# anshumang/gunrockINST

Measured on AMD Instinct MI355X. Metric: MTEPS (million traversed edges/sec) BFS R-MAT scale-24, higher is better.
Workload: dtype int32; 1 GPU; BFS idempotent direction-optimizing (traversal_mode 2), R-MAT scale-24 (a=.55 b=.2 c=.2 d=.05, 8 pairs/vertex mirrored, seed 0x6772): n=16777216, m=265395436 directed edges; sources: largest-degree + 64 seeded; search_depth_src0=7, max_degree=218420

## Files before the change

gunrockinst_amd/capi.py:

```python
import ctypes as C
import os
import subprocess

import numpy as np

_PKG = os.path.dirname(os.path.abspath(__file__))
LIB_PATH = os.environ.get("GUNROCK_LIB_PATH") or os.path.join(_PKG, "lib", "libgunrock.so")
_LIB = None

VTXID_INT = 0
SIZET_INT = 0
VALUE_INT, VALUE_UINT, VALUE_FLOAT = 0, 1, 2
SRC_MANUALLY, SRC_RANDOMIZE, SRC_LARGEST_DEGREE = 0, 1, 2

i32p = C.POINTER(C.c_int32)


class GunrockDataType(C.Structure):
    _fields_ = [("VTXID_TYPE", C.c_int), ("SIZET_TYPE", C.c_int), ("VALUE_TYPE", C.c_int)]


class GunrockGraph(C.Structure):
    _fields_ = [("num_nodes", C.c_size_t), ("num_edges", C.c_size_t),
                ("row_offsets", C.c_void_p), ("col_indices", C.c_void_p),
# ... 65 lines not shown
    "grx_bfs_set_twc_limit": (C.c_int, [C.c_void_p, C.c_int]),
    "grx_bfs_set_binned_min_edges": (C.c_int, [C.c_void_p, C.c_longlong]),
    "grx_bfs_set_label_deferral": (C.c_int, [C.c_void_p, C.c_int, C.c_int]),
    "grx_bfs_set_option": (C.c_int, [C.c_void_p, C.c_char_p, C.c_double]),
    "grx_bfs_set_cooperative_launch": (C.c_int, [C.c_void_p, C.c_int]),
    "grx_bfs_set_head_pass": (C.c_int, [C.c_void_p, C.c_int, C.c_int]),
    "grx_bfs_reset": (C.c_int, [C.c_void_p, C.c_int, C.c_double]),
    "grx_bfs_enact": (C.c_int, [C.c_void_p, C.c_int, C.c_int, C.c_int, C.POINTER(C.c_float)]),
    "grx_bfs_stats": (C.c_int, [C.c_void_p, C.POINTER(C.c_longlong), C.POINTER(C.c_longlong),
                                C.POINTER(C.c_double), C.POINTER(C.c_longlong), C.POINTER(C.c_double)]),
    "grx_bfs_level_trace": (C.c_int, [C.c_void_p, C.c_int, C.POINTER(C.c_longlong), C.POINTER(C.c_longlong),
                                      C.POINTER(C.c_double), i32p]),
    "grx_bfs_extract": (C.c_int, [C.c_void_p, i32p, i32p]),
    "grx_bfs_device_results": (C.c_int, [C.c_void_p, C.POINTER(C.c_void_p), C.POINTER(C.c_void_p)]),
    "grx_bfs_mask_flushes": (C.c_int, [C.c_void_p, C.POINTER(C.c_longlong)]),
    "grx_bfs_relabel_info": (C.c_int, [C.c_void_p, C.POINTER(C.c_longlong), C.POINTER(C.c_longlong), C.POINTER(C.c_int),
                                       C.POINTER(C.c_float), C.POINTER(C.c_longlong)]),
    "grx_bfs_destroy": (None, [C.c_void_p]),
    "grx_cc_create": (C.c_int, [C.POINTER(C.c_void_p), C.c_int, C.c_int]),
    "grx_cc_init": (C.c_int, [C.c_void_p, C.c_int, C.c_int, i32p, i32p]),
    "grx_cc_init_device": (C.c_int, [C.c_void_p, C.c_int, C.c_int, C.c_void_p, C.c_void_p]),
    "grx_cc_reset": (C.c_int, [C.c_void_p]),
    "grx_cc_enact": (C.c_int, [C.c_void_p, C.c_int, C.POINTER(C.c_float)]),
    "grx_cc_stats": (C.c_int, [C.c_void_p, C.POINTER(C.c_longlong), C.POINTER(C.c_longlong), C.POINTER(C.c_longlong),
                               C.POINTER(C.c_double)]),
    "grx_cc_mirrored": (C.c_int, [C.c_void_p, C.POINTER(C.c_int)]),
    "grx_cc_sweep_edges": (C.c_int, [C.c_void_p, C.POINTER(C.c_longlong)]),
    "grx_cc_extract": (C.c_int, [C.c_void_p, i32p, C.POINTER(C.c_uint)]),
    "grx_cc_device_results": (C.c_int, [C.c_void_p, C.POINTER(C.c_void_p)]),
    "grx_cc_destroy": (None, [C.c_void_p]),
# ... 370 lines not shown
        labels = np.empty(max(self.nodes, 1), dtype=np.int32)
        preds = np.empty(max(self.nodes, 1), dtype=np.int32) if self.mark_pred else None
        _check(lib().grx_bfs_extract(self._h, _p(labels), None if preds is None else _p(preds)), "BFSProblem::Extract")
        return labels[:self.nodes], (None if preds is None else preds[:self.nodes])

    def device_results(self):
        dl, dp = C.c_void_p(), C.c_void_p()
        _check(lib().grx_bfs_device_results(self._h, C.byref(dl), C.byref(dp)), "grx_bfs_device_results")
        return dl.value, dp.value

    def mask_flushes(self):
        v = C.c_longlong()
        _check(lib().grx_bfs_mask_flushes(self._h, C.byref(v)), "grx_bfs_mask_flushes")
        return v.value

    def relabel_info(self):
        h, we, t, ms, b = C.c_longlong(), C.c_longlong(), C.c_int(), C.c_float(), C.c_longlong()
        _check(lib().grx_bfs_relabel_info(self._h, C.byref(h), C.byref(we), C.byref(t), C.byref(ms), C.byref(b)),
               "grx_bfs_relabel_info")
        return {"hubs": h.value, "with_edges": we.value, "threshold": t.value, "build_ms": ms.value, "bytes": b.value}


def _graph_struct(nodes, row_offsets, col_indices, edge_values=None):
    g = GunrockGraph()
    g.num_nodes = nodes
    g.num_edges = col_indices.shape[0]
    g.row_offsets = row_offsets.ctypes.data
    g.col_indices = col_indices.ctypes.data
    g.edge_values = None if edge_values is None else edge_values.ctypes.data
    return g
# ... 862 lines not shown
```

gunrockinst_amd/csrc/gunrock/app/bfs/bfs_enactor.hpp:

```cpp
#pragma once

#include <hip/hip_runtime.h>
#include <cstdlib>

#include <gunrock/app/bfs/bfs_functor.hpp>
#include <gunrock/app/bfs/bfs_problem.hpp>
#include <gunrock/app/enactor_base.hpp>
#include <gunrock/oprtr/advance/bottom_up.hpp>
#include <gunrock/oprtr/advance/kernel.hpp>
#include <gunrock/oprtr/advance/twc.hpp>
#include <gunrock/util/context.hpp>

namespace gunrock {
namespace app {
namespace bfs {

template <bool INSTRUMENT>
class BFSEnactor : public EnactorBase {
   public:
    explicit BFSEnactor(bool DEBUG = false) : EnactorBase(VERTEX_FRONTIERS, DEBUG) {}
    ~BFSEnactor() override {}

    void GetKernelStatistics(long long &launches, double &kernel_ms)
    {
        launches = enactor_stats.kernel_launches;
        kernel_ms = enactor_stats.kernel_ms;
    }

    const std::vector<EnactorStats::LevelRecord> &GetLevelTrace() const { return enactor_stats.levels; }

    void GetStatistics(long long &total_queued, long long &search_depth, double &avg_duty)
    {
        total_queued = enactor_stats.total_queued;
        search_depth = enactor_stats.iteration;
        avg_duty = (enactor_stats.total_lifetimes > 0) ? enactor_stats.total_runtimes / enactor_stats.total_lifetimes : 0.0;
    }
    template <typename T>
    void GetStatistics(long long &total_queued, T &search_depth, double &avg_duty)
    {
        long long depth;
        GetStatistics(total_queued, depth, avg_duty);
        search_depth = static_cast<T>(depth);
    }

// ... 32 lines not shown
        hipError_t retval = hipSuccess;
        GraphSlice<VertexId, SizeT, Value> *gs = problem->graph_slices[0];
        oprtr::advance::TailArgs<VertexId, SizeT> t;
        t.queue[0] = gs->frontier_queues[0];
        t.queue[1] = gs->frontier_queues[1];
        t.selector = selector;
        t.first_iteration = iteration;
        t.d_tail = work_progress.d_tail;
        t.edge_limit = problem->tail_edge_limit;
        t.max_levels = kTailMaxLevels;
        t.d_levels_done = work_progress.LevelsDone();
        t.d_level_sums = work_progress.d_sums;
        t.d_row_offsets = gs->d_row_offsets;
        t.d_column_indices = gs->d_column_indices;
        t.d_overflow = work_progress.d_overflow;
        if (twc) {
            t.edge_limit = problem->twc_edge_limit;
            if ((retval = oprtr::advance::LaunchTwcLevels<BFSProblem, BfsFunctor>(t, *problem->data_slices[0], stream))) return retval;
        } else if (persistent) {
            oprtr::advance::PersistentArgs<VertexId, SizeT> p;
            p.t = t;
            long long grid = (static_cast<long long>(queue_edges) + PersistentPolicy::TILE - 1) / PersistentPolicy::TILE;
            if (grid < 16) grid = 16;
            if (grid > cu_count || frontier_size_unknown) grid = cu_count;
            long long limit = grid * PersistentPolicy::TILE * 8;
            if (grid == cu_count || limit > problem->persistent_edge_limit) limit = problem->persistent_edge_limit;
            if (frontier_size_unknown) limit *= 4;
            p.t.edge_limit = static_cast<SizeT>(limit);
            p.barrier.d_counter = work_progress.BarrierCounter();
            p.barrier.d_timeout = work_progress.BarrierTimeout();
            p.solo_edges = problem->tail_edge_limit / 4;
            p.unexplored_edges = unexplored_edges;
            p.switch_factor = switch_factor;
            if ((retval = oprtr::advance::LaunchPersistentLevels<PersistentPolicy, BFSProblem, BfsFunctor>(
                     p, *problem->data_slices[0], cu_count, static_cast<int>(grid), stream, problem->cooperative_launch)))
                return retval;
        } else if ((retval = oprtr::advance::LaunchTailLevels<TailPolicy, BFSProblem, BfsFunctor>(t, *problem->data_slices[0],
                                                                                                   stream)))
            return retval;
        if (closing && (retval = problem->EmitLabelsSpeculative(stream))) return retval;
        if (INSTRUMENT && (retval = InstrumentEnd(stream))) return retval;
        if ((retval = work_progress.GetAll(stream))) return retval;
        if (persistent && work_progress.HostBarrierTimedOut())
            return util::GRError(hipErrorLaunchTimeOut, "BFSEnactor persistent levels kernel: grid barrier timed out", __FILE__,
                                 __LINE__);
        const int done = work_progress.HostLevelsDone();
        iteration += done;
        selector ^= (done & 1);
        queue_length = util::TailCount(work_progress.h_tail[iteration & 3]);
        queue_edges = util::TailEdges(work_progress.h_tail[iteration & 3]);
        if (queue_length > 0) problem->emit_current = false;
        enactor_stats.total_queued += static_cast<long long>(work_progress.h_sums[0]);
        enactor_stats.total_edges_queued += static_cast<long long>(work_progress.h_sums[1]);
        unexplored_edges -= static_cast<long long>(work_progress.h_sums[1]);
        return retval;
    }

    template <typename AdvancePolicy, typename BFSProblem>
    hipError_t EnactBFS(BFSProblem *problem, typename BFSProblem::VertexId src, int max_grid_size, bool dobfs,
                        bool persistent_levels)
    {
        typedef typename BFSProblem::VertexId VertexId;
        typedef typename BFSProblem::SizeT SizeT;
        typedef typename BFSProblem::Value Value;
        typedef BFSFunctor<VertexId, SizeT, Value, BFSProblem> BfsFunctor;
        constexpr int BU_THREADS = 256;

        hipError_t retval = hipSuccess;
        if ((retval = EnactorBase::Setup(max_grid_size, AdvancePolicy::MIN_BLOCKS, 8))) return retval;

        GraphSlice<VertexId, SizeT, Value> *gs = problem->graph_slices[0];
        typename BFSProblem::DataSlice *ds = problem->data_slices[0];
        hipStream_t stream = gs->stream;
        if (src < 0 || src >= problem->nodes) return problem->FinishSearch(stream);
        const bool deferring = dobfs && problem->labels_deferred;
        ds->defer_labels = deferring ? 1 : 0;

        unsigned queue_length = problem->SourceDegree() > 0 ? 1u : 0u;
        unsigned queue_edges = static_cast<unsigned>(problem->SourceDegree());
        if (problem->armed_progress == &work_progress) {
            work_progress.box->overflow = 0;
            problem->armed_progress = nullptr;
        } else if ((retval = work_progress.ResetWithTail(0, queue_length, queue_edges, stream)))
            return retval;
        problem->arm_progress = &work_progress;
        if (INSTRUMENT && (retval = DutyBegin(stream))) return retval;

#ifndef GRX_CONV_GRID_MULT
#define GRX_CONV_GRID_MULT 2
#endif
        const int conv_grid = cu_count * GRX_CONV_GRID_MULT;
        const size_t mask_bytes = sizeof(unsigned) * static_cast<size_t>(problem->MaskWords() + 2);
        long long unexplored_edges = problem->edges;
        bool bottom_up = false;
        bool force_bottom_up = false;
        bool queue_emitted = false;
// ... 143 lines not shown
                if (walk_queue)
                    hipLaunchKernelGGL((oprtr::advance::BottomUpAutoKernel<BU_THREADS, 8, 32, BFSProblem, L, true>), dim3(static_cast<unsigned>(grid)),
                                       dim3(BU_THREADS), 0, stream, bargs, level_slice, lookup, chain, static_cast<unsigned>(sparse_grid),
                                       static_cast<unsigned>(emit_grid));
                else
                    hipLaunchKernelGGL((oprtr::advance::BottomUpAutoKernel<BU_THREADS, 8, 32, BFSProblem, L, false>), dim3(static_cast<unsigned>(grid)),
                                       dim3(BU_THREADS), 0, stream, bargs, level_slice, lookup, chain, static_cast<unsigned>(sparse_grid),
                                       static_cast<unsigned>(emit_grid));
                if ((rc = util::GRError("BottomUpAutoKernel launch failed", __FILE__, __LINE__))) return rc;
                queued = k;
            }
            if (queued == 0) return util::GRError(hipErrorInvalidValue, "BFSEnactor: no frontier bitmap for a bottom-up sweep", __FILE__, __LINE__);
            const bool closing_queued = problem->chain_closing && problem->persistent_edge_limit > 0;
            int *d_gate = work_progress.d_chain_log + 8;
            bool emit_queued = false;
            if (closing_queued) {
                oprtr::advance::PersistentArgs<VertexId, SizeT> p;
                p.t.queue[0] = gs->frontier_queues[0];
                p.t.queue[1] = gs->frontier_queues[1];
                p.t.selector = selector;
                p.t.first_iteration = it0;
                p.t.d_tail = work_progress.d_tail;
                p.t.max_levels = kTailMaxLevels;
                p.t.d_levels_done = work_progress.LevelsDone();
                p.t.d_level_sums = work_progress.d_sums;
                p.t.d_row_offsets = gs->d_row_offsets;
                p.t.d_column_indices = gs->d_column_indices;
                p.t.d_overflow = work_progress.d_overflow;
                p.t.edge_limit = static_cast<SizeT>(static_cast<long long>(problem->persistent_edge_limit) * 4);
                p.barrier.d_counter = work_progress.BarrierCounter();
                p.barrier.d_timeout = work_progress.BarrierTimeout();
                p.solo_edges = problem->tail_edge_limit / 4;
                p.unexplored_edges = unexplored_edges;
                p.switch_factor = 0.0;
                oprtr::advance::SweepChain chain;
                chain.d_sets = work_progress.d_wide;
                chain.base_total = base_total;
                chain.first_in = first_in;
                chain.rule = sweep_rule;
                chain.index = queued;
                chain.first_may_switch = 0;
                chain.d_log = work_progress.d_chain_log;
                if ((rc = oprtr::advance::LaunchChainedPersistentLevels<PersistentPolicy, BFSProblem, BfsFunctor>(
                         p, *ds, cu_count, chain, queued, it0, reinterpret_cast<const int *>(work_progress.AuxTail()), d_gate, stream)))
                    return rc;
                if (deferring && problem->speculative_emit && problem->level_masks.count + queued <= app::bfs::kLevelMasks) {
                    VertexId labels[oprtr::advance::kChainMax];
                    for (int k = 1; k <= queued; ++k) labels[k - 1] = static_cast<VertexId>(it0 + k);
                    if ((rc = problem->EmitLabelsGated(stream, masks + 1, labels, queued, d_gate))) return rc;
                    emit_queued = true;
                }
            }
            if (INSTRUMENT && (rc = InstrumentEnd(stream))) return rc;
            if ((rc = work_progress.Sync(stream))) return rc;
            long long total = base_total;
            int ran = 0, last_action = oprtr::advance::kSweepStop;
            long long next_in = 0;
            for (int k = 1; k <= queued + 1; ++k) {
                const long long in_k = (k == 1 && first_in >= 0) ? first_in
                    : static_cast<long long>(util::TailCount(k == 1 ? work_progress.box->wide : work_progress.box->wide_set[k - 1]));
                next_in = in_k;
                if (k > queued) break;
                const int action = sweep_rule.Decide(in_k, total + in_k, k > 1);
                if (action != work_progress.box->chain_log[k])
                    return util::GRError(hipErrorUnknown, "BFSEnactor: host and device disagree about a chained sweep", __FILE__, __LINE__);
                if (action <= oprtr::advance::kSweepSwitch) break;
                total += in_k;
                ran = k;
                last_action = action;
// ... 330 lines not shown
```

gunrockinst_amd/csrc/gunrock/app/bfs/bfs_problem.hpp:

```cpp
#pragma once

#include <hip/hip_runtime.h>

#include <gunrock/app/problem_base.hpp>
#include <gunrock/graphio/device_csr.hpp>
#include <gunrock/graphio/relabel.hpp>
#include <gunrock/oprtr/advance/binned.hpp>
#include <gunrock/oprtr/advance/bottom_up.hpp>
#include <gunrock/util/memset_kernel.hpp>

namespace gunrock {
namespace app {
namespace bfs {

template <typename SizeT>
__global__ void NoInEdgeMaskKernel(const SizeT *d_inv_row_offsets, long long nodes, long long words64, unsigned long long *d_mask)
{
    const unsigned lane = threadIdx.x & 63;
    const long long wave0 = (static_cast<long long>(blockIdx.x) * blockDim.x + threadIdx.x) / 64;
    const long long nwaves = static_cast<long long>(gridDim.x) * blockDim.x / 64;
    for (long long w = wave0; w < words64; w += nwaves) {
        const long long v = w * 64 + lane;
        const bool none = v < nodes && d_inv_row_offsets[v + 1] == d_inv_row_offsets[v];
        const unsigned long long m = __ballot(none);
// ... 818 lines not shown
        GR_CHECK(hipStreamSynchronize(stream), "BFSProblem Extract sync failed");
        if (this->nodes > 0)
            GR_CHECK(hipMemcpy(h_labels, d_out_labels, sizeof(VertexId) * static_cast<size_t>(this->nodes), hipMemcpyDeviceToHost),
                     "BFSProblem hipMemcpy d_labels failed");
        if (MARK_PREDECESSORS && h_preds && this->nodes > 0)
            GR_CHECK(hipMemcpy(h_preds, d_out_preds, sizeof(VertexId) * static_cast<size_t>(this->nodes), hipMemcpyDeviceToHost),
                     "BFSProblem hipMemcpy d_preds failed");
        return retval;
    }

    bool defer_labels = true;
    bool emit_current = false;
    bool labels_deferred = false;
    int label_pass = 1;
    int walk_queue = 1;
    int level_mask_limit = kLevelMasks;
    LevelMaskList<VertexId> level_masks;
    int mask_ring = 0;

    bool MaskKept(int idx) const
    {
        for (int k = 0; k < level_masks.count; ++k)
            if (level_masks.mask[k] == reinterpret_cast<const unsigned long long *>(data_slices[0]->d_frontier_mask[idx])) return true;
        return false;
    }
    hipError_t AcquireMask(hipStream_t stream, int &idx, int hold_a = -1, int hold_b = -1)
    {
        const int holds[2] = {hold_a, hold_b};
        bool got = false;
        const hipError_t rc = TryAcquireMask(stream, idx, holds, 2, got);
// ... 163 lines not shown
```

gunrockinst_amd/csrc/gunrock/oprtr/advance/kernel.hpp:

```cpp
#pragma once

#include <hip/hip_runtime.h>
#include <cstdlib>
#include <climits>
#include <limits>
#include <type_traits>

#include <gunrock/oprtr/advance/binned.hpp>
#include <gunrock/oprtr/advance/functor_hooks.hpp>
#include <gunrock/oprtr/advance/sweep_chain.hpp>
#include <gunrock/oprtr/frontier_writer.hpp>
#include <gunrock/util/device_intrinsics.hpp>
#include <gunrock/util/error_utils.hpp>
#include <gunrock/util/frontier.hpp>
#include <gunrock/util/kernel_runtime_stats.hpp>

namespace gunrock {
namespace oprtr {
namespace advance {

enum MODE { TWC_FORWARD, TWC_BACKWARD, LB_BACKWARD, LB };
enum TYPE { V2V, V2E, E2V, E2E };
enum REDUCE_OP { NONE, PLUS, MINUS, MULTIPLIES, MODULUS, BIT_OR, BIT_AND, BIT_XOR, MAXIMUM, MINIMUM };
enum REDUCE_TYPE { EMPTY, VERTEX, EDGE };
// ... 489 lines not shown
}

template <typename VertexId, typename SizeT>
struct TailArgs {
    util::Frontier<VertexId, SizeT> queue[2];
    int selector;
    long long first_iteration;
    unsigned long long *d_tail;
    SizeT edge_limit;
    int max_levels;
    int *d_levels_done;
    unsigned long long *d_level_sums;
    const SizeT *d_row_offsets;
    const VertexId *d_column_indices;
    int *d_overflow;
};

template <typename KernelPolicy, typename ProblemData, typename Functor>
__global__ __launch_bounds__(KernelPolicy::THREADS) void TailLevelsKernel(
    TailArgs<typename ProblemData::VertexId, typename ProblemData::SizeT> t, typename ProblemData::DataSlice slice)
{
    typedef typename ProblemData::VertexId VertexId;
    typedef typename ProblemData::SizeT SizeT;
    typedef AdvanceShared<KernelPolicy, VertexId, SizeT> Shared;
    typedef typename Shared::Writer Writer;
    __shared__ Shared sh;

    Writer::Init(sh.writer);
    unsigned tile_tag;
    InitOwnerMarks<KernelPolicy>(sh, tile_tag);
    int selector = t.selector;
// ... 25 lines not shown

        const long long tiles = (static_cast<long long>(edges) + KernelPolicy::TILE - 1) / KernelPolicy::TILE;
        unsigned accepted = 0;
        ExpandTiles<KernelPolicy, ProblemData, Functor, true, true>(a, slice, 0, tiles, sh, accepted, tile_tag);
        const int rest = Writer::Count(sh.writer);
        __syncthreads();
        Writer::template Flush<true>(sh.writer, rest, a.out, a.d_tail_out, a.d_overflow, a.d_row_offsets);
        asm volatile("s_waitcnt vmcnt(0)" ::: "memory");
        __syncthreads();
        selector ^= 1;
        ++iteration;
        ++done;
        sum_len += len;
        sum_edges += edges;
    }
    if (threadIdx.x == 0) {
        *t.d_levels_done = done;
        t.d_level_sums[0] = sum_len;
        t.d_level_sums[1] = sum_edges;
    }
}

template <typename KernelPolicy, typename ProblemData, typename Functor, bool OUT_WITH_DEGREES = true, bool COUNT_ONLY = false>
hipError_t LaunchKernel(const AdvanceArgs<typename ProblemData::VertexId, typename ProblemData::SizeT> &args,
                        const typename ProblemData::DataSlice &slice, int max_grid_size, hipStream_t stream,
                        TYPE  = V2V)
{
    if (args.in_len <= 0 || args.in_edges <= 0) return hipSuccess;
    const long long tiles = (static_cast<long long>(args.in_edges) + KernelPolicy::TILE - 1) / KernelPolicy::TILE;
    if (max_grid_size <= 0)
        max_grid_size = util::ResidentGrid(LoadBalancedKernel<KernelPolicy, ProblemData, Functor, OUT_WITH_DEGREES, COUNT_ONLY>, KernelPolicy::THREADS);
    long long grid = tiles < max_grid_size ? tiles : max_grid_size;
    if (grid < 1) grid = 1;
    hipLaunchKernelGGL((LoadBalancedKernel<KernelPolicy, ProblemData, Functor, OUT_WITH_DEGREES, COUNT_ONLY>), dim3(static_cast<unsigned>(grid)),
                       dim3(KernelPolicy::THREADS), 0, stream, args, slice);
// ... 173 lines not shown
            __syncthreads();
            Writer::template Flush<true>(sh.writer, rest, a.out, a.d_tail_out, a.d_overflow, a.d_row_offsets);
        }
        if (solo) {
            asm volatile("s_waitcnt vmcnt(0)" ::: "memory");
            __syncthreads();
        } else if (!GridBarrier(p.barrier, epoch))
            break;
        selector ^= 1;
        ++iteration;
        ++done;
        sum_len += len;
        sum_edges += edges;
        unexplored -= edges;
    }
    if (blockIdx.x == 0 && threadIdx.x == 0) {
        *t.d_levels_done = done;
        t.d_level_sums[0] = sum_len;
        t.d_level_sums[1] = sum_edges;
    }
}

template <typename KernelPolicy, typename ProblemData, typename Functor>
__global__ __launch_bounds__(KernelPolicy::THREADS) void PersistentLevelsKernel(
    PersistentArgs<typename ProblemData::VertexId, typename ProblemData::SizeT> p, typename ProblemData::DataSlice slice)
{
    PersistentLevelsBody<KernelPolicy, ProblemData, Functor>(p, slice, p.t.first_iteration);
}

template <typename KernelPolicy, typename ProblemData, typename Functor>
__global__ __launch_bounds__(KernelPolicy::THREADS) void ChainedPersistentLevelsKernel(
    PersistentArgs<typename ProblemData::VertexId, typename ProblemData::SizeT> p, typename ProblemData::DataSlice slice,
    SweepChain chain, int sweeps, long long first_level, const int *d_queue_invalid, int *d_gate)
{
    const ChainEnd end = ChainOutcome(chain, sweeps, util::LaneId());
    const bool run = end.action == kSweepSwitch && end.end >= 2 && end.prev_action == kSweepSparseEmit && *d_queue_invalid == 0;
    if (blockIdx.x == 0 && threadIdx.x == 0) {
        d_gate[0] = run ? 1 : 0;
        d_gate[1] = end.end - 1;
        if (!run) {
            *p.t.d_levels_done = 0;
            p.t.d_level_sums[0] = 0ull;
            p.t.d_level_sums[1] = 0ull;
        }
    }
    if (!run) return;
    PersistentLevelsBody<KernelPolicy, ProblemData, Functor>(p, slice, first_level + (end.end - 1));
}

template <typename KernelPolicy, typename ProblemData, typename Functor>
hipError_t LaunchPersistentLevels(const PersistentArgs<typename ProblemData::VertexId, typename ProblemData::SizeT> &args,
                                  const typename ProblemData::DataSlice &slice, int cu_count, int grid_hint, hipStream_t stream,
                                  bool cooperative = false)
{
    int grid = util::ResidentGrid(PersistentLevelsKernel<KernelPolicy, ProblemData, Functor>, KernelPolicy::THREADS);
    if (grid > cu_count) grid = cu_count;
    if (grid_hint > 0 && grid_hint < grid) grid = grid_hint;
    if (grid < 1) grid = 1;
    if (cooperative) {
        PersistentArgs<typename ProblemData::VertexId, typename ProblemData::SizeT> a = args;
        typename ProblemData::DataSlice s = slice;
// ... 36 lines not shown
```

gunrockinst_amd/csrc/gunrock/util/frontier.hpp:

```cpp
#pragma once

#include <hip/hip_runtime.h>
#include <set>
#include <cstdint>
#include <cstring>

#include <gunrock/util/error_utils.hpp>

namespace gunrock {
namespace util {

template <typename VertexId, typename SizeT>
struct Frontier {
    VertexId *v = nullptr;
    SizeT *row_start = nullptr;
    SizeT *scan = nullptr;
    SizeT capacity = 0;
};

__host__ __device__ __forceinline__ unsigned long long PackTail(unsigned count, unsigned edges)
{
    return (static_cast<unsigned long long>(edges) << 32) | count;
}
__host__ __device__ __forceinline__ unsigned TailCount(unsigned long long t) { return static_cast<unsigned>(t); }
// ... 11 lines not shown
{
    return d_wide ? d_wide + (blockIdx.x & 31u) * 16u : nullptr;
}

struct HostMailbox {
    unsigned long long seq;
    unsigned long long tail[8];
    unsigned long long sums[2];
    unsigned long long wide;
    unsigned long long overflow;
    unsigned long long set_value;
    unsigned long long wide_set[8];
    int chain_log[8];
};

static __global__ void PublishKernel(unsigned long long *d_tail, const unsigned long long *d_sums, unsigned long long *d_wide,
                                     const int *d_overflow, HostMailbox *box, unsigned long long seq, unsigned clear_mask,
                                     unsigned ones_mask, int wide_sets, const int *d_chain_log)
{
    const unsigned lane = threadIdx.x;
    if (lane < 8) {
        const unsigned long long v = d_tail[lane];
        box->tail[lane] = v;
        if (lane == 7 || ((clear_mask >> lane) & 1u)) d_tail[lane] = 0ull;
        else if ((ones_mask >> lane) & 1u) d_tail[lane] = ~0ull;
    }
    if (lane < 2) box->sums[lane] = d_sums[lane];
    unsigned long long w = 0;
    if (lane < 32) {
        w = d_wide[lane * 16];
        if (w) d_wide[lane * 16] = 0;
    }
    for (int o = 16; o; o >>= 1) w += __shfl_xor(w, o, 64);
    if (lane == 0) {
        box->wide = w;
        box->overflow = static_cast<unsigned long long>(*d_overflow);
    }
    if (wide_sets > 1) {
        unsigned long long ws[7];
#pragma unroll
        for (int k = 1; k < 8; ++k) ws[k - 1] = (k < wide_sets && lane < 32) ? d_wide[k * 512 + lane * 16] : 0ull;
#pragma unroll
        for (int k = 1; k < 8; ++k) {
            if (k < wide_sets) {
                if (ws[k - 1]) d_wide[k * 512 + lane * 16] = 0ull;
                unsigned long long t = ws[k - 1];
                for (int o = 16; o; o >>= 1) t += __shfl_xor(t, o, 64);
                if (lane == 0) box->wide_set[k] = t;
            }
        }
        if (lane < 8) box->chain_log[lane] = d_chain_log[lane];
    }
    __threadfence_system();
    __syncthreads();
    if (lane == 0) __hip_atomic_store(&box->seq, seq, __ATOMIC_RELEASE, __HIP_MEMORY_SCOPE_SYSTEM);
}

static __global__ void ArmKernel(unsigned long long *d_tail, int *d_overflow, unsigned long long *d_wide, int slots, int wide_lines,
                                 int wide_stride, int seed_slot, unsigned long long seed_value, int wide_sets)
{
    const int lane = threadIdx.x;
    if (lane < slots) d_tail[lane] = (lane == seed_slot) ? seed_value : 0ull;
    if (lane < wide_lines)
        for (int k = 0; k < wide_sets; ++k) d_wide[(k * wide_lines + lane) * wide_stride] = 0ull;
    if (lane == 0) *d_overflow = 0;
}

struct WorkProgress {
    static constexpr int kSlots = 8;
    static constexpr int kAux = 4;
    unsigned long long *d_tail = nullptr;
    int *d_overflow = nullptr;
    unsigned long long *d_sums = nullptr;
    static constexpr int kWideLines = 32;
    static constexpr int kWideStride = 16;
    static constexpr int kWideSets = 8;
    static constexpr int kWideSetWords = kWideLines * kWideStride;
    unsigned long long *d_wide = nullptr;
    int *d_chain_log = nullptr;
    int publish_sets = 1;
    HostMailbox *box = nullptr;
    unsigned long long *h_sums = nullptr;
    unsigned long long *h_tail = nullptr;
    unsigned long long seq = 0;

    static std::set<const WorkProgress *> &Live()
    {
        static std::set<const WorkProgress *> *live = new std::set<const WorkProgress *>();
        return *live;
    }
    static bool IsLive(const WorkProgress *p) { return p && Live().count(p) != 0; }

    hipError_t Init()
    {
        hipError_t retval = hipSuccess;
        if (d_tail) return retval;
        Live().insert(this);
        GR_CHECK(hipMalloc(&d_tail, sizeof(unsigned long long) * kSlots), "WorkProgress hipMalloc d_tail failed");
        GR_CHECK(hipMalloc(&d_overflow, sizeof(int)), "WorkProgress hipMalloc d_overflow failed");
// ... 15 lines not shown
    }

    hipError_t Reset(hipStream_t stream)
    {
        hipError_t retval = hipSuccess;
        GR_CHECK(hipMemsetAsync(d_tail, 0, sizeof(unsigned long long) * kSlots, stream), "WorkProgress memset failed");
        GR_CHECK(hipMemsetAsync(d_overflow, 0, sizeof(int), stream), "WorkProgress memset failed");
        GR_CHECK(hipMemsetAsync(d_wide, 0, sizeof(unsigned long long) * kWideSets * kWideSetWords, stream),
                 "WorkProgress memset failed");
        return retval;
    }

    hipError_t ResetWithTail(int slot, unsigned count, unsigned edges, hipStream_t stream)
    {
        box->overflow = 0;
        hipLaunchKernelGGL(ArmKernel, dim3(1), dim3(64), 0, stream, d_tail, d_overflow, d_wide, kSlots, kWideLines, kWideStride, slot & 3,
                           PackTail(count, edges), kWideSets);
        return GRError(hipGetLastError(), "WorkProgress ArmKernel launch failed", __FILE__, __LINE__);
    }

    hipError_t SetTail(int slot, unsigned count, unsigned edges, hipStream_t stream)
    {
        box->set_value = PackTail(count, edges);
        box->overflow = 0;
        return GRError(hipMemcpyAsync(d_tail + (slot & 3), &box->set_value, sizeof(unsigned long long), hipMemcpyHostToDevice, stream),
                       "WorkProgress SetTail failed", __FILE__, __LINE__);
    }

    hipError_t Sync(hipStream_t stream, unsigned clear_mask = 0, unsigned ones_mask = 0)
    {
        hipError_t retval = hipSuccess;
        ++seq;
        hipLaunchKernelGGL(PublishKernel, dim3(1), dim3(64), 0, stream, d_tail, d_sums, d_wide, d_overflow, box, seq, clear_mask,
                           ones_mask, publish_sets, d_chain_log);
        GR_CHECK(hipGetLastError(), "WorkProgress PublishKernel launch failed");
        volatile unsigned long long *flag = &box->seq;
        unsigned spins = 0;
        while (__atomic_load_n(flag, __ATOMIC_ACQUIRE) != seq) {
            if ((++spins & 0x3FFu) == 0) {
                hipError_t rc = hipStreamQuery(stream);
                if (rc == hipSuccess) {
                    if (__atomic_load_n(flag, __ATOMIC_ACQUIRE) == seq) break;
                    continue;
                }
                if (rc != hipErrorNotReady) return GRError(rc, "WorkProgress Sync: stream failed", __FILE__, __LINE__);
            }
        }
        return retval;
    }

    hipError_t GetTail(int slot, unsigned &count, unsigned &edges, hipStream_t stream)
    {
        hipError_t retval = hipSuccess;
        GR_CHECK(Sync(stream), "WorkProgress GetTail sync failed");
        count = TailCount(h_tail[slot & 3]);
        edges = TailEdges(h_tail[slot & 3]);
        return retval;
    }

    hipError_t GetTailWide(int slot, unsigned &count, unsigned &edges, hipStream_t stream)
    {
        hipError_t retval = hipSuccess;
        GR_CHECK(Sync(stream), "WorkProgress GetTailWide sync failed");
        count = TailCount(h_tail[slot & 3]) + TailCount(box->wide);
        edges = TailEdges(h_tail[slot & 3]) + TailEdges(box->wide);
// ... 53 lines not shown
```

gunrockinst_amd/csrc/lib/bfs_app.hip:

```cpp
#include <gunrock/gunrock.h>
#include <gunrock/gunrock_mi355x.h>

#include <cstdio>
#include <cstdlib>

#include <gunrock/app/bfs/bfs_enactor.hpp>
#include <gunrock/app/bfs/bfs_problem.hpp>
#include <gunrock/app/handle_runner.hpp>
#include <gunrock/graphio/device_sort.hpp>
#include <gunrock/graphio/symmetry.hpp>
#include <gunrock/oprtr/filter/kernel.hpp>
#include <gunrock/csr.hpp>
#include <gunrock/graphio/utils.hpp>
#include <gunrock/util/context.hpp>

using namespace gunrock;
using namespace gunrock::app;
using namespace gunrock::app::bfs;

namespace {

struct BfsRunner {
    virtual ~BfsRunner() {}
    virtual hipError_t Init(const Csr<int, int, int> &g) = 0;
// ... 4 lines not shown
    virtual void SetPersistentLimit(int limit) = 0;
    virtual void SetTwcLimit(int limit) = 0;
    virtual void SetCooperativeLaunch(bool on) = 0;
    virtual void SetBinnedMinEdges(long long min_edges) = 0;
    virtual void SetLabelDeferral(int enabled, int mask_limit) = 0;
    virtual int SetOption(const char *name, double value) = 0;
    virtual void SetHeadPass(int min_edges, int max_edges) = 0;
    virtual hipError_t Reset(int src, double queue_sizing) = 0;
    virtual hipError_t Enact(int src, int max_grid_size, int traversal_mode, float *ms) = 0;
    virtual void Stats(long long &queued, long long &depth, double &duty, long long &launches, double &kernel_ms) = 0;
    virtual int Trace(int max_levels, long long *frontier, long long *edges, double *ms, int *kind) = 0;
    virtual hipError_t Extract(int *labels, int *preds) = 0;
    virtual void DeviceResults(int **labels, int **preds) = 0;
    virtual void BuildRelabelled(bool on) = 0;
    virtual long long MaskFlushes() = 0;
    virtual void RelabelInfo(long long &hubs, long long &with_edges, int &threshold, float &build_ms, long long &bytes) = 0;
};

template <bool PRED, bool IDEMP, bool INSTR>
struct BfsRunnerT : BfsRunner {
    typedef BFSProblem<int, int, int, PRED, IDEMP, (PRED && IDEMP)> Problem;
    util::DeviceContext context;
    Problem problem;
    BFSEnactor<INSTR> enactor;
    EventPair timer;

    explicit BfsRunnerT(int device) : context(device), enactor(false) { timer.Create(); }
    ~BfsRunnerT() override { FreeInverse(); }
    hipError_t Init(const Csr<int, int, int> &g) override { return problem.Init(false, g, 1); }
    hipError_t InitDevice(int nodes, int edges, int *d_ro, int *d_ci) override
// ... 51 lines not shown
    int *d_inv_column_indices = nullptr;
    void SetPersistentLimit(int limit) override { problem.persistent_edge_limit = limit; }
    void SetTwcLimit(int limit) override { problem.twc_edge_limit = limit; }
    void SetCooperativeLaunch(bool on) override { problem.cooperative_launch = on; }
    void SetBinnedMinEdges(long long min_edges) override { problem.binned_min_edges = min_edges; }
    int SetOption(const char *name, double value) override
    {
        const std::string key(name ? name : "");
        if (key == "emit_queue_factor") problem.emit_queue_factor = static_cast<float>(value);
        else if (key == "sparse_sweep_div") problem.sparse_sweep_div = static_cast<int>(value);
        else if (key == "speculative_emit") problem.speculative_emit = value != 0.0;
        else if (key == "chain_sweeps") problem.chain_sweeps = static_cast<int>(value);
        else if (key == "chain_closing") problem.chain_closing = value != 0.0;
        else if (key == "label_pass") problem.label_pass = value != 0.0 ? 1 : 0;
        else if (key == "walk_queue") problem.walk_queue = value != 0.0 ? 1 : 0;
        else if (key == "relabel") {
            if (value > 0.0 && !problem.HasRelabelled()) return 2;
            problem.relabel = value > 0.0 ? 1 : (value < 0.0 ? -1 : 0);
        } else if (key == "relabel_min_nodes") {
            if (value < 0.0) return 2;
            problem.relabel_min_nodes = static_cast<long long>(value);
        } else if (key == "relabel_hubs") {
            if (value < 0.0) return 2;
            const long long hubs = static_cast<long long>(value);
            if (!problem.HasRelabelled()) problem.relabel_hubs = hubs;
            else if (hubs != problem.relabel_hubs && problem.BuildRelabelled(hubs) != hipSuccess) return 3;
        } else return 1;
        return 0;
    }
    void BuildRelabelled(bool on) override { problem.build_relabelled = on; }
    long long MaskFlushes() override { return problem.mask_flushes; }
    void RelabelInfo(long long &hubs, long long &with_edges, int &threshold, float &build_ms, long long &bytes) override
    {
        const bool ready = problem.HasRelabelled();
        hubs = ready ? problem.relabelled.hubs : -1;
        with_edges = ready ? problem.relabelled.with_edges : -1;
        threshold = ready ? problem.relabelled.threshold : 0;
        build_ms = ready ? problem.relabelled.build_ms : 0.f;
        const long long n = problem.nodes, words = (n + 63) / 64 + 2;
        bytes = ready ? static_cast<long long>(problem.relabelled.bytes) + words * 8 + (words + 1) * 4 + n * 8 + n * 4 * (problem.MARK_PREDECESSORS ? 2 : 1) : 0;
    }
    void SetLabelDeferral(int enabled, int mask_limit) override
    {
        if (enabled >= 0) problem.defer_labels = enabled != 0;
        if (mask_limit > 0) problem.level_mask_limit = mask_limit;
    }
// ... 217 lines not shown
    if (!p || !h_labels) return -1;
    return static_cast<int>(p->runner->Extract(h_labels, h_preds));
}

int grx_bfs_device_results(grx_bfs *p, int **d_labels, int **d_preds)
{
    if (!p) return -1;
    p->runner->DeviceResults(d_labels, d_preds);
    return 0;
}

int grx_bfs_mask_flushes(grx_bfs *p, long long *flushes)
{
    if (!p || !p->runner || !flushes) return -1;
    *flushes = p->runner->MaskFlushes();
    return 0;
}

int grx_bfs_relabel_info(grx_bfs *p, long long *hubs, long long *with_edges, int *threshold, float *build_ms, long long *bytes)
{
    if (!p || !p->runner) return -1;
    long long h = -1, we = -1, b = 0;
    int t = 0;
    float ms = 0.f;
    p->runner->RelabelInfo(h, we, t, ms, b);
    if (hubs) *hubs = h;
    if (with_edges) *with_edges = we;
    if (threshold) *threshold = t;
    if (build_ms) *build_ms = ms;
    if (bytes) *bytes = b;
// ... 103 lines not shown
```

include/gunrock/gunrock_mi355x.h:

```cpp
#ifndef GUNROCK_GUNROCK_MI355X_H_
#define GUNROCK_GUNROCK_MI355X_H_

#include <stddef.h>
#include <stdint.h>

#ifdef __cplusplus
extern "C" {
#endif

typedef struct grx_graph grx_graph;

int grx_graph_from_market(const char *path, int undirected, int reversed, grx_graph **out);
int grx_graph_from_market_cached(const char *path, int undirected, int reversed, int *cache_hit, grx_graph **out);
int grx_graph_rmat_libc(int nodes, int edges, int undirected, double a, double b, double c, double d, grx_graph **out);
int grx_graph_rmat_seeded(int scale, long long pairs, uint64_t seed, int undirected,
                          double a, double b, double c, double d, grx_graph **out);
int grx_graph_from_coo(int nodes, long long tuples, const int *rows, const int *cols, const int *vals, grx_graph **out);
int grx_graph_from_csr(int nodes, int edges, const int *row_offsets, const int *col_indices, const int *edge_values,
                       grx_graph **out);
int grx_graph_nodes(const grx_graph *g);
int grx_graph_edges(const grx_graph *g);
const int *grx_graph_row_offsets(const grx_graph *g);
const int *grx_graph_col_indices(const grx_graph *g);
const int *grx_graph_edge_values(const grx_graph *g);
// ... 15 lines not shown

int grx_bfs_create(grx_bfs **out, int mark_pred, int idempotence, int instrument, int device);
int grx_bfs_init(grx_bfs *p, int nodes, int edges, const int *row_offsets, const int *col_indices);
int grx_bfs_init_device(grx_bfs *p, int nodes, int edges, int *d_row_offsets, int *d_col_indices);
int grx_bfs_set_inverse_graph(grx_bfs *p, const int *d_inv_row_offsets, const int *d_inv_col_indices,
                              float alpha, float beta);
int grx_bfs_auto_inverse(grx_bfs *p, int build_if_directed, int *enabled, int *built, float *build_ms);
int grx_bfs_set_tuning(grx_bfs *p, float alpha, float beta, float lite_factor, int tail_edge_limit);
int grx_bfs_set_persistent_limit(grx_bfs *p, int edge_limit);
int grx_bfs_set_twc_limit(grx_bfs *p, int edge_limit);
int grx_bfs_set_cooperative_launch(grx_bfs *p, int on);
int grx_bfs_set_binned_min_edges(grx_bfs *p, long long min_edges);
int grx_bfs_set_label_deferral(grx_bfs *p, int enabled, int mask_limit);
int grx_bfs_set_option(grx_bfs *p, const char *name, double value);
int grx_bfs_mask_flushes(grx_bfs *p, long long *flushes);
int grx_bfs_relabel_info(grx_bfs *p, long long *hubs, long long *with_edges, int *threshold, float *build_ms, long long *bytes);
int grx_bfs_set_head_pass(grx_bfs *p, int min_edges, int max_edges);
int grx_bfs_reset(grx_bfs *p, int src, double queue_sizing);
int grx_bfs_enact(grx_bfs *p, int src, int max_grid_size, int traversal_mode, float *elapsed_ms);
int grx_bfs_stats(grx_bfs *p, long long *total_queued, long long *search_depth, double *avg_duty,
                  long long *kernel_launches, double *kernel_ms);
int grx_bfs_level_trace(grx_bfs *p, int max_levels, long long *frontier, long long *edges, double *ms, int *kind);
int grx_bfs_extract(grx_bfs *p, int *h_labels, int *h_preds);
int grx_bfs_device_results(grx_bfs *p, int **d_labels, int **d_preds);
void grx_bfs_destroy(grx_bfs *p);
int grx_filter_queue(int n, const int *d_in, const int *d_row_offsets, int capacity, int *d_out_v, int *d_out_row_start, int *d_out_scan,
                     int *out_len, long long *out_edges, int max_grid_size);

enum grx_advance_mode { GRX_ADVANCE_IDS = 0, GRX_ADVANCE_FRONTIER = 1, GRX_ADVANCE_COUNT_ONLY = 2 };
enum grx_advance_rule { GRX_ADVANCE_RULE_MASK = 0, GRX_ADVANCE_RULE_CLAIM = 1 };
// ... 193 lines not shown
```

Before: 1.022 million MTEPS.

## Publish level counters from inside tail kernels instead of separate publish launch

The tail, persistent and chained-persistent level kernels now write their final counters, wide sums and overflow flag directly into the host-mapped mailbox. The host then spins on the mailbox sequence number instead of launching a separate PublishKernel and synchronizing the stream. This removes one kernel launch and a stream sync per host readback on the tail path. In exchange it adds barrier re-arming via a memset, a polling fallback to a full sync, and overflow handling that zeros the queue. Readback counters are exposed for diagnostics.

Result: no change. 1.021 million MTEPS (-0.1%).

```diff
diff --git a/gunrockinst_amd/capi.py b/gunrockinst_amd/capi.py
--- a/gunrockinst_amd/capi.py
+++ b/gunrockinst_amd/capi.py
@@ -103,6 +103,7 @@
     "grx_bfs_extract": (C.c_int, [C.c_void_p, i32p, i32p]),
     "grx_bfs_device_results": (C.c_int, [C.c_void_p, C.POINTER(C.c_void_p), C.POINTER(C.c_void_p)]),
     "grx_bfs_mask_flushes": (C.c_int, [C.c_void_p, C.POINTER(C.c_longlong)]),
+    "grx_bfs_readback_counts": (C.c_int, [C.c_void_p, C.POINTER(C.c_longlong), C.POINTER(C.c_longlong)]),
     "grx_bfs_relabel_info": (C.c_int, [C.c_void_p, C.POINTER(C.c_longlong), C.POINTER(C.c_longlong), C.POINTER(C.c_int),
                                        C.POINTER(C.c_float), C.POINTER(C.c_longlong)]),
     "grx_bfs_destroy": (None, [C.c_void_p]),
@@ -503,6 +504,11 @@
         _check(lib().grx_bfs_mask_flushes(self._h, C.byref(v)), "grx_bfs_mask_flushes")
         return v.value
 
+    def readback_counts(self):
+        launches, fallbacks = C.c_longlong(), C.c_longlong()
+        _check(lib().grx_bfs_readback_counts(self._h, C.byref(launches), C.byref(fallbacks)), "grx_bfs_readback_counts")
+        return launches.value, fallbacks.value
+
     def relabel_info(self):
         h, we, t, ms, b = C.c_longlong(), C.c_longlong(), C.c_int(), C.c_float(), C.c_longlong()
         _check(lib().grx_bfs_relabel_info(self._h, C.byref(h), C.byref(we), C.byref(t), C.byref(ms), C.byref(b)),
diff --git a/gunrockinst_amd/csrc/gunrock/app/bfs/bfs_enactor.hpp b/gunrockinst_amd/csrc/gunrock/app/bfs/bfs_enactor.hpp
--- a/gunrockinst_amd/csrc/gunrock/app/bfs/bfs_enactor.hpp
+++ b/gunrockinst_amd/csrc/gunrock/app/bfs/bfs_enactor.hpp
@@ -28,6 +28,12 @@
     }
 
     const std::vector<EnactorStats::LevelRecord> &GetLevelTrace() const { return enactor_stats.levels; }
+
+    void GetReadbackCounts(long long &publish_launches, long long &fallbacks) const
+    {
+        publish_launches = work_progress.publish_launches;
+        fallbacks = work_progress.publish_fallbacks;
+    }
 
     void GetStatistics(long long &total_queued, long long &search_depth, double &avg_duty)
     {
@@ -90,6 +96,8 @@
         t.d_row_offsets = gs->d_row_offsets;
         t.d_column_indices = gs->d_column_indices;
         t.d_overflow = work_progress.d_overflow;
+        const bool inline_publish = !twc && UseInlinePublish(problem);
+        if (inline_publish) ArmInlinePublish(t);
         if (twc) {
             t.edge_limit = problem->twc_edge_limit;
             if ((retval = oprtr::advance::LaunchTwcLevels<BFSProblem, BfsFunctor>(t, *problem->data_slices[0], stream))) return retval;
@@ -108,6 +116,8 @@
             p.solo_edges = problem->tail_edge_limit / 4;
             p.unexplored_edges = unexplored_edges;
             p.switch_factor = switch_factor;
+            if ((retval = work_progress.RearmBarrier(stream))) return retval;
+            work_progress.barrier_dirty = inline_publish;
             if ((retval = oprtr::advance::LaunchPersistentLevels<PersistentPolicy, BFSProblem, BfsFunctor>(
                      p, *problem->data_slices[0], cu_count, static_cast<int>(grid), stream, problem->cooperative_launch)))
                 return retval;
@@ -116,7 +126,7 @@
             return retval;
         if (closing && (retval = problem->EmitLabelsSpeculative(stream))) return retval;
         if (INSTRUMENT && (retval = InstrumentEnd(stream))) return retval;
-        if ((retval = work_progress.GetAll(stream))) return retval;
+        if ((retval = inline_publish ? work_progress.WaitPublished(stream) : work_progress.GetAll(stream))) return retval;
         if (persistent && work_progress.HostBarrierTimedOut())
             return util::GRError(hipErrorLaunchTimeOut, "BFSEnactor persistent levels kernel: grid barrier timed out", __FILE__,
                                  __LINE__);
@@ -129,7 +139,27 @@
         enactor_stats.total_queued += static_cast<long long>(work_progress.h_sums[0]);
         enactor_stats.total_edges_queued += static_cast<long long>(work_progress.h_sums[1]);
         unexplored_edges -= static_cast<long long>(work_progress.h_sums[1]);
+        if (work_progress.OverflowAtLastSync()) {
+            queue_length = 0;
+            queue_edges = 0;
+        }
         return retval;
+    }
+
+    template <typename BFSProblem>
+    bool UseInlinePublish(const BFSProblem *problem) const
+    {
+        return !INSTRUMENT && problem->inline_publish != 0;
+    }
+    template <typename VertexId, typename SizeT>
+    void ArmInlinePublish(oprtr::advance::TailArgs<VertexId, SizeT> &t)
+    {
+        t.publish = 1;
+        t.publish_sets = work_progress.publish_sets;
+        t.publish_seq = work_progress.NextSeq();
+        t.box = work_progress.box;
+        t.d_wide = work_progress.d_wide;
+        t.d_chain_log = work_progress.d_chain_log;
     }
 
     template <typename AdvancePolicy, typename BFSProblem>
@@ -156,6 +186,7 @@
         unsigned queue_edges = static_cast<unsigned>(problem->SourceDegree());
         if (problem->armed_progress == &work_progress) {
             work_progress.box->overflow = 0;
+            work_progress.barrier_dirty = false;
             problem->armed_progress = nullptr;
         } else if ((retval = work_progress.ResetWithTail(0, queue_length, queue_edges, stream)))
             return retval;
@@ -329,6 +360,7 @@
             const bool closing_queued = problem->chain_closing && problem->persistent_edge_limit > 0;
             int *d_gate = work_progress.d_chain_log + 8;
             bool emit_queued = false;
+            const bool inline_publish = closing_queued && UseInlinePublish(problem);
             if (closing_queued) {
                 oprtr::advance::PersistentArgs<VertexId, SizeT> p;
                 p.t.queue[0] = gs->frontier_queues[0];
@@ -356,6 +388,9 @@
                 chain.index = queued;
                 chain.first_may_switch = 0;
                 chain.d_log = work_progress.d_chain_log;
+                if (inline_publish) ArmInlinePublish(p.t);
+                if ((rc = work_progress.RearmBarrier(stream))) return rc;
+                work_progress.barrier_dirty = inline_publish;
                 if ((rc = oprtr::advance::LaunchChainedPersistentLevels<PersistentPolicy, BFSProblem, BfsFunctor>(
                          p, *ds, cu_count, chain, queued, it0, reinterpret_cast<const int *>(work_progress.AuxTail()), d_gate, stream)))
                     return rc;
@@ -367,7 +402,7 @@
                 }
             }
             if (INSTRUMENT && (rc = InstrumentEnd(stream))) return rc;
-            if ((rc = work_progress.Sync(stream))) return rc;
+            if ((rc = inline_publish ? work_progress.WaitPublished(stream) : work_progress.Sync(stream))) return rc;
             long long total = base_total;
             int ran = 0, last_action = oprtr::advance::kSweepStop;
             long long next_in = 0;
diff --git a/gunrockinst_amd/csrc/gunrock/app/bfs/bfs_problem.hpp b/gunrockinst_amd/csrc/gunrock/app/bfs/bfs_problem.hpp
--- a/gunrockinst_amd/csrc/gunrock/app/bfs/bfs_problem.hpp
+++ b/gunrockinst_amd/csrc/gunrock/app/bfs/bfs_problem.hpp
@@ -856,6 +856,7 @@
     bool labels_deferred = false;
     int label_pass = 1;
     int walk_queue = 1;
+    int inline_publish = 1;
     int level_mask_limit = kLevelMasks;
     LevelMaskList<VertexId> level_masks;
     int mask_ring = 0;
diff --git a/gunrockinst_amd/csrc/gunrock/oprtr/advance/kernel.hpp b/gunrockinst_amd/csrc/gunrock/oprtr/advance/kernel.hpp
--- a/gunrockinst_amd/csrc/gunrock/oprtr/advance/kernel.hpp
+++ b/gunrockinst_amd/csrc/gunrock/oprtr/advance/kernel.hpp
@@ -527,7 +527,31 @@
     const SizeT *d_row_offsets;
     const VertexId *d_column_indices;
     int *d_overflow;
+    int publish = 0;
+    int publish_sets = 1;
+    unsigned long long publish_seq = 0;
+    util::HostMailbox *box = nullptr;
+    unsigned long long *d_wide = nullptr;
+    const int *d_chain_log = nullptr;
 };
+
+template <typename VertexId, typename SizeT>
+__device__ __forceinline__ void FinishLevels(const TailArgs<VertexId, SizeT> &t, int done, unsigned long long sum_len,
+                                             unsigned long long sum_edges)
+{
+    if (t.publish) {
+        asm volatile("s_waitcnt vmcnt(0)" ::: "memory");
+        __syncthreads();
+    }
+    if (threadIdx.x == 0) {
+        *t.d_levels_done = done;
+        t.d_level_sums[0] = sum_len;
+        t.d_level_sums[1] = sum_edges;
+    }
+    if (t.publish && threadIdx.x < util::kWaveSize)
+        util::PublishWords<true>(t.d_tail, t.d_level_sums, t.d_wide, t.d_overflow, t.box, t.publish_seq, 0u, 0u, t.publish_sets,
+                                 t.d_chain_log, threadIdx.x, done, sum_len, sum_edges);
+}
 
 template <typename KernelPolicy, typename ProblemData, typename Functor>
 __global__ __launch_bounds__(KernelPolicy::THREADS) void TailLevelsKernel(
@@ -583,11 +607,7 @@
         sum_len += len;
         sum_edges += edges;
     }
-    if (threadIdx.x == 0) {
-        *t.d_levels_done = done;
-        t.d_level_sums[0] = sum_len;
-        t.d_level_sums[1] = sum_edges;
-    }
+    FinishLevels(t, done, sum_len, sum_edges);
 }
 
 template <typename KernelPolicy, typename ProblemData, typename Functor, bool OUT_WITH_DEGREES = true, bool COUNT_ONLY = false>
@@ -791,11 +811,7 @@
         sum_edges += edges;
         unexplored -= edges;
     }
-    if (blockIdx.x == 0 && threadIdx.x == 0) {
-        *t.d_levels_done = done;
-        t.d_level_sums[0] = sum_len;
-        t.d_level_sums[1] = sum_edges;
-    }
+    if (blockIdx.x == 0) FinishLevels(t, done, sum_len, sum_edges);
 }
 
 template <typename KernelPolicy, typename ProblemData, typename Functor>
@@ -815,13 +831,11 @@
     if (blockIdx.x == 0 && threadIdx.x == 0) {
         d_gate[0] = run ? 1 : 0;
         d_gate[1] = end.end - 1;
-        if (!run) {
-            *p.t.d_levels_done = 0;
-            p.t.d_level_sums[0] = 0ull;
-            p.t.d_level_sums[1] = 0ull;
-        }
-    }
-    if (!run) return;
+    }
+    if (!run) {
+        if (blockIdx.x == 0) FinishLevels(p.t, 0, 0ull, 0ull);
+        return;
+    }
     PersistentLevelsBody<KernelPolicy, ProblemData, Functor>(p, slice, first_level + (end.end - 1));
 }
 
diff --git a/gunrockinst_amd/csrc/gunrock/util/frontier.hpp b/gunrockinst_amd/csrc/gunrock/util/frontier.hpp
--- a/gunrockinst_amd/csrc/gunrock/util/frontier.hpp
+++ b/gunrockinst_amd/csrc/gunrock/util/frontier.hpp
@@ -49,32 +49,41 @@
     int chain_log[8];
 };
 
-static __global__ void PublishKernel(unsigned long long *d_tail, const unsigned long long *d_sums, unsigned long long *d_wide,
-                                     const int *d_overflow, HostMailbox *box, unsigned long long seq, unsigned clear_mask,
-                                     unsigned ones_mask, int wide_sets, const int *d_chain_log)
-{
-    const unsigned lane = threadIdx.x;
+template <bool AGENT, typename T>
+__device__ __forceinline__ T PublishLoad(const T *p)
+{
+    if (AGENT) return __hip_atomic_load(p, __ATOMIC_RELAXED, __HIP_MEMORY_SCOPE_AGENT);
+    return *p;
+}
+
+template <bool IN_KERNEL>
+__device__ __forceinline__ void PublishWords(unsigned long long *d_tail, const unsigned long long *d_sums, unsigned long long *d_wide,
+                                             const int *d_overflow, HostMailbox *box, unsigned long long seq, unsigned clear_mask,
+                                             unsigned ones_mask, int wide_sets, const int *d_chain_log, unsigned lane,
+                                             int levels_done = 0, unsigned long long sum_len = 0ull, unsigned long long sum_edges = 0ull)
+{
     if (lane < 8) {
-        const unsigned long long v = d_tail[lane];
+        unsigned long long v = PublishLoad<IN_KERNEL>(d_tail + lane);
+        if (IN_KERNEL && lane == 6) v = (v & 0xFFFFFFFF00000000ull) | static_cast<unsigned>(levels_done);
         box->tail[lane] = v;
-        if (lane == 7 || ((clear_mask >> lane) & 1u)) d_tail[lane] = 0ull;
+        if ((!IN_KERNEL && lane == 7) || ((clear_mask >> lane) & 1u)) d_tail[lane] = 0ull;
         else if ((ones_mask >> lane) & 1u) d_tail[lane] = ~0ull;
     }
-    if (lane < 2) box->sums[lane] = d_sums[lane];
+    if (lane < 2) box->sums[lane] = IN_KERNEL ? (lane == 0 ? sum_len : sum_edges) : d_sums[lane];
     unsigned long long w = 0;
     if (lane < 32) {
-        w = d_wide[lane * 16];
+        w = PublishLoad<IN_KERNEL>(d_wide + lane * 16);
         if (w) d_wide[lane * 16] = 0;
     }
     for (int o = 16; o; o >>= 1) w += __shfl_xor(w, o, 64);
     if (lane == 0) {
         box->wide = w;
-        box->overflow = static_cast<unsigned long long>(*d_overflow);
+        box->overflow = static_cast<unsigned long long>(PublishLoad<IN_KERNEL>(d_overflow));
     }
     if (wide_sets > 1) {
         unsigned long long ws[7];
 #pragma unroll
-        for (int k = 1; k < 8; ++k) ws[k - 1] = (k < wide_sets && lane < 32) ? d_wide[k * 512 + lane * 16] : 0ull;
+        for (int k = 1; k < 8; ++k) ws[k - 1] = (k < wide_sets && lane < 32) ? PublishLoad<IN_KERNEL>(d_wide + k * 512 + lane * 16) : 0ull;
 #pragma unroll
         for (int k = 1; k < 8; ++k) {
             if (k < wide_sets) {
@@ -84,11 +93,17 @@
                 if (lane == 0) box->wide_set[k] = t;
             }
         }
-        if (lane < 8) box->chain_log[lane] = d_chain_log[lane];
+        if (lane < 8) box->chain_log[lane] = PublishLoad<IN_KERNEL>(d_chain_log + lane);
     }
     __threadfence_system();
-    __syncthreads();
     if (lane == 0) __hip_atomic_store(&box->seq, seq, __ATOMIC_RELEASE, __HIP_MEMORY_SCOPE_SYSTEM);
+}
+
+static __global__ void PublishKernel(unsigned long long *d_tail, const unsigned long long *d_sums, unsigned long long *d_wide,
+                                     const int *d_overflow, HostMailbox *box, unsigned long long seq, unsigned clear_mask,
+                                     unsigned ones_mask, int wide_sets, const int *d_chain_log)
+{
+    PublishWords<false>(d_tail, d_sums, d_wide, d_overflow, box, seq, clear_mask, ones_mask, wide_sets, d_chain_log, threadIdx.x);
 }
 
 static __global__ void ArmKernel(unsigned long long *d_tail, int *d_overflow, unsigned long long *d_wide, int slots, int wide_lines,
@@ -118,6 +133,9 @@
     unsigned long long *h_sums = nullptr;
     unsigned long long *h_tail = nullptr;
     unsigned long long seq = 0;
+    long long publish_launches = 0;
+    long long publish_fallbacks = 0;
+    bool barrier_dirty = false;
 
     static std::set<const WorkProgress *> &Live()
     {
@@ -163,6 +181,7 @@
     hipError_t ResetWithTail(int slot, unsigned count, unsigned edges, hipStream_t stream)
     {
         box->overflow = 0;
+        barrier_dirty = false;
         hipLaunchKernelGGL(ArmKernel, dim3(1), dim3(64), 0, stream, d_tail, d_overflow, d_wide, kSlots, kWideLines, kWideStride, slot & 3,
                            PackTail(count, edges), kWideSets);
         return GRError(hipGetLastError(), "WorkProgress ArmKernel launch failed", __FILE__, __LINE__);
@@ -180,6 +199,8 @@
     {
         hipError_t retval = hipSuccess;
         ++seq;
+        ++publish_launches;
+        barrier_dirty = false;
         hipLaunchKernelGGL(PublishKernel, dim3(1), dim3(64), 0, stream, d_tail, d_sums, d_wide, d_overflow, box, seq, clear_mask,
                            ones_mask, publish_sets, d_chain_log);
         GR_CHECK(hipGetLastError(), "WorkProgress PublishKernel launch failed");
@@ -198,6 +219,31 @@
         return retval;
     }
 
+    unsigned long long NextSeq() { return ++seq; }
+    hipError_t WaitPublished(hipStream_t stream)
+    {
+        volatile unsigned long long *flag = &box->seq;
+        unsigned spins = 0;
+        while (__atomic_load_n(flag, __ATOMIC_ACQUIRE) != seq) {
+            if ((++spins & 0x3FFu) == 0) {
+                hipError_t rc = hipStreamQuery(stream);
+                if (rc == hipSuccess) {
+                    if (__atomic_load_n(flag, __ATOMIC_ACQUIRE) == seq) break;
+                    ++publish_fallbacks;
+                    return Sync(stream);
+                }
+                if (rc != hipErrorNotReady) return GRError(rc, "WorkProgress WaitPublished: stream failed", __FILE__, __LINE__);
+            }
+        }
+        return hipSuccess;
+    }
+    hipError_t RearmBarrier(hipStream_t stream)
+    {
+        if (!barrier_dirty) return hipSuccess;
+        barrier_dirty = false;
+        return GRError(hipMemsetAsync(d_tail + 7, 0, sizeof(unsigned long long), stream), "WorkProgress RearmBarrier failed", __FILE__, __LINE__);
+    }
+
     hipError_t GetTail(int slot, unsigned &count, unsigned &edges, hipStream_t stream)
     {
         hipError_t retval = hipSuccess;
diff --git a/gunrockinst_amd/csrc/lib/bfs_app.hip b/gunrockinst_amd/csrc/lib/bfs_app.hip
--- a/gunrockinst_amd/csrc/lib/bfs_app.hip
+++ b/gunrockinst_amd/csrc/lib/bfs_app.hip
@@ -42,6 +42,7 @@
     virtual void DeviceResults(int **labels, int **preds) = 0;
     virtual void BuildRelabelled(bool on) = 0;
     virtual long long MaskFlushes() = 0;
+    virtual void ReadbackCounts(long long &publish_launches, long long &fallbacks) = 0;
     virtual void RelabelInfo(long long &hubs, long long &with_edges, int &threshold, float &build_ms, long long &bytes) = 0;
 };
 
@@ -123,6 +124,7 @@
         else if (key == "chain_closing") problem.chain_closing = value != 0.0;
         else if (key == "label_pass") problem.label_pass = value != 0.0 ? 1 : 0;
         else if (key == "walk_queue") problem.walk_queue = value != 0.0 ? 1 : 0;
+        else if (key == "inline_publish") problem.inline_publish = value != 0.0 ? 1 : 0;
         else if (key == "relabel") {
             if (value > 0.0 && !problem.HasRelabelled()) return 2;
             problem.relabel = value > 0.0 ? 1 : (value < 0.0 ? -1 : 0);
@@ -139,6 +141,7 @@
     }
     void BuildRelabelled(bool on) override { problem.build_relabelled = on; }
     long long MaskFlushes() override { return problem.mask_flushes; }
+    void ReadbackCounts(long long &publish_launches, long long &fallbacks) override { enactor.GetReadbackCounts(publish_launches, fallbacks); }
     void RelabelInfo(long long &hubs, long long &with_edges, int &threshold, float &build_ms, long long &bytes) override
     {
         const bool ready = problem.HasRelabelled();
@@ -386,6 +389,16 @@
 {
     if (!p || !p->runner || !flushes) return -1;
     *flushes = p->runner->MaskFlushes();
+    return 0;
+}
+
+int grx_bfs_readback_counts(grx_bfs *p, long long *publish_launches, long long *fallbacks)
+{
+    if (!p || !p->runner) return -1;
+    long long launches = 0, fb = 0;
+    p->runner->ReadbackCounts(launches, fb);
+    if (publish_launches) *publish_launches = launches;
+    if (fallbacks) *fallbacks = fb;
     return 0;
 }
 
diff --git a/include/gunrock/gunrock_mi355x.h b/include/gunrock/gunrock_mi355x.h
--- a/include/gunrock/gunrock_mi355x.h
+++ b/include/gunrock/gunrock_mi355x.h
@@ -53,6 +53,7 @@
 int grx_bfs_set_label_deferral(grx_bfs *p, int enabled, int mask_limit);
 int grx_bfs_set_option(grx_bfs *p, const char *name, double value);
 int grx_bfs_mask_flushes(grx_bfs *p, long long *flushes);
+int grx_bfs_readback_counts(grx_bfs *p, long long *publish_launches, long long *fallbacks);
 int grx_bfs_relabel_info(grx_bfs *p, long long *hubs, long long *with_edges, int *threshold, float *build_ms, long long *bytes);
 int grx_bfs_set_head_pass(grx_bfs *p, int min_edges, int max_edges);
 int grx_bfs_reset(grx_bfs *p, int src, double queue_sizing);
```
